# domargan/parallel-packed-csr

Hardware: AMD Instinct MI355X
Metric: edge-updates/sec (higher is better)
Workload: dtype u32; 1 GPU; config#2 1000000 random inserts on RMAT scale-20 / 10000000-edge core, 1 partition, labels raw; vertices=1048576, core_edges=10000000, parallelism=1 partition(s), 1 per GPU x 1 GPU(s), logN=32, distinct_update_batches=4, semantics=sequential stream order (bit-exact vs reference -threads=1)

## Files before the change

### parallel-packed-csr_amd/csrc/engine.cc

```cpp
#include "engine.h"

#include <stdio.h>
#include <stdlib.h>

#include <algorithm>
#include <map>
#include <memory>
#include <vector>
#include <chrono>

#include "gpu_rt.h"
#define GPU_DFREE(x) gpu::dfree_named((x), #x, __LINE__)
#include "pma_kernels.h"

namespace ppcsr {

#define GCHK(expr)                                                                       \
  do {                                                                                   \
    int _e = (expr);                                                                     \
    if (_e != 0) return fail(PPCSR_EHIP, std::string(#expr) + ": " + gpu::err_str(_e)); \
  } while (0)

struct DevGuard {
  std::vector<void **> slots;
// ... 39 lines not shown
  uint64_t rank_cap = 0, tiles_cap = 0;
  unsigned long long *d_total = nullptr, *h_total = nullptr;
  ChainTable *d_table = nullptr;
  unsigned long long *d_scan_state = nullptr;
  uint64_t scan_state_cap = 0, scan_nchunks = 0;
  Edge *d_scratch = nullptr;
  uint64_t scratch_cap = 0;
  int *d_nbr = nullptr;
  uint64_t nbr_cap = 0;
  uint32_t round = 0;
  uint32_t max_horizon = 4096, min_horizon = 64, rounds_per_sync = 32, init_horizon = 256;
  gpu::Timer timer;
  EngineStats st{};
  struct Snap {
    View v{};
    uint64_t cap_slots = 0, cap_nodes = 0;
    bool valid = false;
    uint32_t synced = 0;
    uint64_t gen = 0;
  };
  Snap snap, esnap;
  uint32_t snap_grid = 4096;
  bool snap_count = false;
  uint64_t snap_ctr[6] = {0, 0, 0, 0, 0, 0};
  unsigned long long *d_snapcnt = nullptr;
  uint64_t scc_ctr[8] = {0, 0, 0, 0, 0, 0, 0, 0};
  uint64_t msf_ctr[8] = {0, 0, 0, 0, 0, 0, 0, 0};
  uint64_t ktruss_ctr[8] = {0, 0, 0, 0, 0, 0, 0, 0};
  uint64_t msbfs_ctr[8] = {0, 0, 0, 0, 0, 0, 0, 0};
  uint32_t msbfs_look = 1;
  uint32_t serial = 1;
  uint64_t array_gen = 1;
  bool stamps_clean = false;
  OptCtl *d_octl = nullptr, *h_octl = nullptr;
  uint32_t *d_vdbg = nullptr;
  uint32_t *d_status = nullptr, *d_carry0 = nullptr, *d_carry1 = nullptr;
  uint64_t carry_cap = 0, hslot_cap = 0;
  unsigned long long *d_regfail = nullptr, *d_pfail = nullptr;
  uint32_t *d_vws = nullptr, *d_vrs = nullptr;
  uint32_t *d_wstamp = nullptr, *d_rstamp = nullptr;
  uint32_t mode = 1;
  uint32_t epoch_ops = 1u << 20;
  uint32_t cur_epoch = 0;
  uint32_t epoch_short = 16384;
  uint32_t epoch_clean = 0, epoch_grow_after = 2;
  uint32_t epoch_adapt = 8, grow_eff = 2;
  uint64_t since_rollback = 0;
  double rb_dist = -1.0;
  uint32_t region_slots = 1024;
  uint32_t region_wide = 4096, region_calm = 8, region_eff = 0, region_clean = 0;
  uint32_t region_rare = 16384, region_rare_calm = 8, region_rare_dist = 65536;
  uint64_t region_rare_span = 0;
  uint32_t region_rare_cpr = 1536;
  double cpr_mean = -1.0;
  uint32_t resident_waves = 0;
  uint32_t opt_horizon = 6144;
  uint32_t start_horizon = 6144;
  uint32_t adaptive = 1;
  uint32_t rb_defer_table = 1u << 22;
  uint32_t scatter_blocks = 8192;
  uint32_t small_batch = 256;
  uint32_t excl_in_wave = 4096;
  uint32_t big_window = 32768, big_min = 256, big_grid = 64;
  dev::BigJob *d_jobs = nullptr;
  Edge *d_bigscratch = nullptr;
  uint64_t bigscratch_cap = 0;
// ... 479 lines not shown
  }
  if (k == "rb_prefetch") {
    p.rb_prefetch = value ? 1u : 0u;
    return PPCSR_OK;
  }
  if (k == "msbfs_look") {
    p.msbfs_look = value ? 1u : 0u;
    return PPCSR_OK;
  }
  if (k == "scatter_variant") {
    p.scatter_variant = value > 2 ? 2u : (uint32_t)value;
    return PPCSR_OK;
  }
  if (k == "adaptive") {
    p.adaptive = value != 0;
    return PPCSR_OK;
  }
  if (k == "resident_waves") {
    if (value < 0 || value > (1 << 20)) return fail(PPCSR_EINVAL, "resident_waves out of range");
    p.resident_waves = (uint32_t)value;
    return PPCSR_OK;
  }
  if (k == "start_horizon") {
    if (value < 1 || value > (1 << 20)) return fail(PPCSR_EINVAL, "start_horizon out of range");
    p.start_horizon = (uint32_t)value;
    return PPCSR_OK;
  }
  if (k == "test_block_rebalance") {
    const uint64_t ws = (uint64_t)value >> 32, wl = (uint64_t)value & 0xFFFFFFFFull;
    if (wl < 64 || (wl & (wl - 1)) || ws % wl || ws + wl > p.v.g.N || (wl >> p.v.g.sh) > dev::kBigLeaves) return fail(PPCSR_EINVAL, "bad window");
    gpu::set_device(device_);
    Edge *sc = nullptr;
    GCHK(gpu::dmalloc((void **)&sc, wl * sizeof(Edge)));
    GPU_LAUNCH(p.stream, k_block_rebalance, 1, dev::kBigThreads, p.v, ws, wl, sc);
    GCHK(gpu::sync(p.stream));
    GCHK(gpu::last_error());
    gpu::dfree(sc);
    return PPCSR_OK;
  }
  if (k == "marker") {
    gpu::set_device(device_);
    uint32_t *np_ = nullptr;
    switch (value) {
      case 0: GPU_LAUNCH(p.stream, k_mark_0, 1, 64, np_); break;
      case 1: GPU_LAUNCH(p.stream, k_mark_1, 1, 64, np_); break;
      case 2: GPU_LAUNCH(p.stream, k_mark_2, 1, 64, np_); break;
      case 3: GPU_LAUNCH(p.stream, k_mark_3, 1, 64, np_); break;
      case 4: GPU_LAUNCH(p.stream, k_mark_4, 1, 64, np_); break;
      case 5: GPU_LAUNCH(p.stream, k_mark_5, 1, 64, np_); break;
      case 6: GPU_LAUNCH(p.stream, k_mark_6, 1, 64, np_); break;
      case 7: GPU_LAUNCH(p.stream, k_mark_7, 1, 64, np_); break;
      default: return fail(PPCSR_EINVAL, "marker id must be 0..7");
    }
    return PPCSR_OK;
  }
  if (k == "epoch_short") {
    p.epoch_short = (uint32_t)std::max<int64_t>(64, value);
    return PPCSR_OK;
  }
  if (k == "epoch_adapt") {
    p.epoch_adapt = (uint32_t)std::max<int64_t>(0, std::min<int64_t>(value, 1024));
    return PPCSR_OK;
  }
  if (k == "epoch_grow_after") {
    p.epoch_grow_after = (uint32_t)std::max<int64_t>(1, value);
    return PPCSR_OK;
// ... 60 lines not shown
    bool &f;
    explicit InBatch(bool &x) : f(x) { f = true; }
    ~InBatch() { f = false; }
  } in_batch_guard(p.in_batch);
  const uint64_t kChunk = 1ull << 30;
  for (uint64_t off = 0; off < n; off += kChunk) {
    const uint64_t m = std::min(kChunk, n - off);
    const bool small = m <= p.small_batch;
    int rc;
    if (p.v.g.narrow == 0u) {
      rc = recheck_ranges();
      if (rc != PPCSR_OK) return rc;
    }
    if (p.v.g.narrow == 0u) {
      const uint32_t mh = p.max_horizon, mi = p.min_horizon, ih = p.init_horizon;
      p.max_horizon = p.min_horizon = p.init_horizon = 1;
      rc = run_rounds(d_ops + off, m);
      p.max_horizon = mh;
      p.min_horizon = mi;
      p.init_horizon = ih;
    } else {
      rc = (p.mode == 1 && !small) ? run_speculative(d_ops + off, m) : run_rounds(d_ops + off, m);
    }
    if (rc != PPCSR_OK) return rc;
  }
  p.timer.stop(p.stream);
  p.st.last_batch_ms = p.timer.ms();
  p.st.ops_applied += n;
  return inplace_fault_check();
}

int Engine::run_rounds(const Op *d_ops, uint64_t n) {
  Impl &p = *p_;
  if (p.round > 0xFFFF0000u) GCHK(reset_tags(p));
  GCHK(ensure_plans(p));
  uint64_t cur = 0;
  uint32_t hor = (uint32_t)std::min<uint64_t>(p.init_horizon, n);
  while (cur < n) {
    const uint32_t par = (p.round + 1) & 1u;
    Control &c = *p.h_ctl;
    c.base[par] = (uint32_t)cur;
    c.base[par ^ 1u] = (uint32_t)cur;
    c.horizon[par] = (uint32_t)std::min<uint64_t>(hor, n - cur);
    c.horizon[par ^ 1u] = 0;
    c.failmin[0] = c.failmin[1] = kMax;
    c.n_ops = (uint32_t)n;
    c.excl = 0;
    c.error = 0;
    c.max_horizon = p.max_horizon;
    c.rounds = c.committed = c.planned = 0;
    GCHK(gpu::h2d(p.d_ctl, p.h_ctl, sizeof(Control), p.stream));
    bool need_excl = false;
    while (cur < n && !need_excl) {
      RoundArgs a;
      a.v = p.v;
      a.ops = d_ops;
      a.plans = p.d_plans;
      a.ctl = p.d_ctl;
      a.stats = p.d_stats;
      a.min_horizon = p.min_horizon;
      const uint32_t blocks = (p.max_horizon + 3) / 4;
      if (p.profile && p.events.size() < 4ull * p.rounds_per_sync) {
        const size_t old = p.events.size();
        p.events.resize(4ull * p.rounds_per_sync);
        for (size_t i = old; i < p.events.size(); i++) GCHK(p.events[i].init());
      }
// ... 21 lines not shown
          p.st.prof_plan_ms += gpu::Event::elapsed_ms(p.events[4 * r + 0], p.events[4 * r + 1]);
          p.st.prof_check_ms += gpu::Event::elapsed_ms(p.events[4 * r + 1], p.events[4 * r + 2]);
          p.st.prof_apply_ms += gpu::Event::elapsed_ms(p.events[4 * r + 2], p.events[4 * r + 3]);
          p.st.prof_launches += 1;
        }
      }
      p.st.round_syncs++;
      if (c.error) return fail(PPCSR_EINTERNAL, "device-side error " + std::to_string(c.error));
      const uint32_t npar = (p.round + 1) & 1u;
      cur = c.base[npar];
      hor = std::max<uint32_t>(c.horizon[npar], p.min_horizon);
      need_excl = c.excl != 0;
      p.st.rounds += c.rounds;
      p.st.committed += c.committed;
      p.st.planned += c.planned;
      c.rounds = c.committed = c.planned = 0;
      if (!need_excl && cur < n) {
        GCHK(gpu::dset(&p.d_ctl->rounds, 0, 3 * sizeof(unsigned long long), p.stream));
      }
    }
    if (need_excl && cur < n) {
      GCHK(gpu::d2h(p.h_op1, d_ops + cur, sizeof(Op), p.stream));
      GCHK(gpu::sync(p.stream));
      int rc = run_exclusive(*p.h_op1, 0);
      if (rc != PPCSR_OK) return rc;
      cur += 1;
    }
  }
  return PPCSR_OK;
}

static int snap_commit(Engine::Impl &p, Engine::Impl::Snap &sn);
static int snap_rollback(Engine::Impl &p, Engine::Impl::Snap &sn, Engine::Impl::Snap &other);

int Engine::run_speculative(const Op *d_ops, uint64_t n) {
  Impl &p = *p_;
  GCHK(ensure_plans(p));
  if (p.hslot_cap < p.opt_horizon) {
    if (p.d_status) GPU_DFREE(p.d_status);
    p.d_status = nullptr;
    p.hslot_cap = 0;
    GCHK(gpu::dmalloc((void **)&p.d_status, ((uint64_t)p.opt_horizon + 64) * sizeof(uint32_t)));
    if (p.d_vdbg) GPU_DFREE(p.d_vdbg);
    GCHK(gpu::dmalloc((void **)&p.d_vdbg, ((uint64_t)p.opt_horizon + 64) * 4 * sizeof(uint32_t)));
    p.hslot_cap = p.opt_horizon;
  }
  const uint64_t carry_need = (uint64_t)p.opt_horizon + 8;
  if (p.carry_cap < carry_need) {
    if (p.d_carry0) GPU_DFREE(p.d_carry0);
    if (p.d_carry1) GPU_DFREE(p.d_carry1);
    p.d_carry0 = p.d_carry1 = nullptr;
    p.carry_cap = 0;
    GCHK(gpu::dmalloc((void **)&p.d_carry0, kStripes * carry_need * sizeof(uint32_t)));
    GCHK(gpu::dmalloc((void **)&p.d_carry1, kStripes * carry_need * sizeof(uint32_t)));
    p.carry_cap = carry_need;
  }
  uint32_t bigw = p.big_window;
  while (bigw > kBigWindow && (bigw >> p.v.g.sh) > dev::kBigLeaves) bigw >>= 1;
  const bool use_big = bigw > p.big_min;
  if (use_big) {
    if (!p.d_jobs) GCHK(gpu::dmalloc((void **)&p.d_jobs, kBigJobs * sizeof(dev::BigJob)));
    const uint64_t need = (uint64_t)p.big_grid * bigw;
    if (p.bigscratch_cap < need) {
      if (p.d_bigscratch) GPU_DFREE(p.d_bigscratch);
      p.d_bigscratch = nullptr;
      p.bigscratch_cap = 0;
      GCHK(gpu::dmalloc((void **)&p.d_bigscratch, need * sizeof(Edge)));
      p.bigscratch_cap = need;
    }
  }
  if (p.diag >= 2) {
    if (p.dg_cap < n) {
      if (p.d_dg) GPU_DFREE(p.d_dg);
      p.d_dg = nullptr;
      p.dg_cap = 0;
      GCHK(gpu::dmalloc((void **)&p.d_dg, n * 4 * sizeof(uint32_t)));
      p.dg_cap = n;
    }
    GCHK(gpu::dset(p.d_dg, 0, n * 4 * sizeof(uint32_t), p.stream));
  }
  p.stamps_clean = false;
  uint64_t e0 = 0;
  uint64_t forced_e1 = 0;
  int retries = 0;
  const uint32_t kEpochShort = p.epoch_short;
  if (p.cur_epoch == 0 || p.cur_epoch > p.epoch_ops) p.cur_epoch = p.epoch_ops;
  while (e0 < n) {
    uint64_t e1 = std::min<uint64_t>(e0 + p.cur_epoch, n);
    if (forced_e1 > e0 && forced_e1 < e1) e1 = forced_e1;
    if (p.round > 0xFFFF0000u) GCHK(reset_tags(p));
    GCHK(snap_commit(p, p.esnap));
    GCHK(gpu::d2d(p.d_stats_snap, p.d_stats, kStatShards * sizeof(StatShard), p.stream));
    if (!p.stamps_clean) {
      const uint64_t leaves = p.v.g.N >> p.v.g.sh;
      GCHK(gpu::dset(p.d_wstamp, 0, leaves * sizeof(uint32_t), p.stream));
      GCHK(gpu::dset(p.d_rstamp, 0, leaves * sizeof(uint32_t), p.stream));
      GCHK(gpu::dset(p.d_vws, 0, (p.n_cap + 1) * sizeof(uint32_t), p.stream));
      GCHK(gpu::dset(p.d_vrs, 0, (p.n_cap + 1) * sizeof(uint32_t), p.stream));
      p.stamps_clean = true;
    }
    OptCtl &c = *p.h_octl;
    memset(&c, 0, sizeof(c));
    const uint32_t pp0 = p.round & 1u;
    c.hor[pp0] = 0;
    c.used[pp0] = 0;
    c.nf[pp0] = (uint32_t)e0;
    c.adaptive = p.adaptive;
    c.cur_h[pp0] = p.adaptive ? std::min(p.start_horizon, p.opt_horizon) : p.opt_horizon;
    c.book_round = p.round;
    for (int t = 0; t < 3; t++) {
      c.minkept[t] = kMax;
      c.gbar[t] = c.sbar[t] = ~0ull;
    }
    c.e1 = (uint32_t)e1;
    c.max_horizon = p.opt_horizon;
    c.width_cap = p.opt_horizon;
    c.resident = p.resident_waves;
    c.viol_idx = kMax;
    c.skip_idx = kMax;
    c.skip_round = 0;
    GCHK(gpu::h2d(p.d_octl, p.h_octl, sizeof(OptCtl), p.stream));
    int rs = 0;
    if (p.region_eff < p.region_slots) p.region_eff = p.region_slots;
    while ((p.region_eff >> rs) > (uint32_t)p.v.g.logN) rs++;
    bool epoch_open = true;
    uint32_t cur_width = c.cur_h[pp0];
    uint64_t carry_now = 0;
    unsigned long long jobs_seen = 0, rounds_seen = 0, planned_seen = 0, long_seen = 0;
    uint64_t chunk_pending = e1 - e0;
    double chunk_cpr = 0.9 * (double)std::min<uint64_t>(cur_width, e1 - e0);
    unsigned long long prev_rounds = 0, prev_committed = 0;
    uint32_t excl_cooldown = 0;
    while (epoch_open) {
      OptArgs a;
      a.v = p.v;
      a.v.big_window = use_big ? bigw : kBigWindow;
      a.big_min = p.big_min;
      a.jobs = use_big ? p.d_jobs : (dev::BigJob *)nullptr;
      a.bigscratch = p.d_bigscratch;
      a.bigscratch_stride = bigw;
      a.ops = d_ops;
      a.plans = p.d_plans;
      a.status = p.d_status;
      a.vdbg = p.d_vdbg;
      a.carry0 = p.d_carry0;
      a.carry1 = p.d_carry1;
      a.carry_cap = (uint32_t)p.carry_cap;
      a.ctl = p.d_octl;
      a.stats = p.d_stats;
      a.regfail = p.d_regfail;
      a.pfail = p.d_pfail;
      a.wstamp = p.d_wstamp;
      a.rstamp = p.d_rstamp;
      a.vws = p.d_vws;
      a.vrs = p.d_vrs;
      a.regshift = rs;
      a.diag = p.diag;
      a.defer_barrier = p.defer_barrier;
      const bool extras = p.diag != 0 || p.dbg_repeat != 0;
      a.dbg = p.dbg_repeat;
      a.dg = p.diag >= 2 ? p.d_dg : (uint32_t *)nullptr;
      a.soft_barrier = p.soft_barrier ? p.soft_barrier : a.v.big_window / 2u;
      if (!p.soft_barrier && p.region_rare_span && p.region_eff >= p.region_rare) a.soft_barrier = 0x40000000u;
      uint32_t gh = p.opt_horizon;
      {
        const uint64_t want = std::max<uint64_t>(1024, 4ull * (cur_width ? cur_width : p.opt_horizon));
        if (want < gh) gh = (uint32_t)want;
        const uint64_t pend = (chunk_pending + 255) & ~255ull;
        if (pend < gh) gh = (uint32_t)std::max<uint64_t>(pend, 256);
        const uint64_t need = (carry_now + 255) & ~255ull;
        if (gh < need) gh = (uint32_t)std::min<uint64_t>(need, p.opt_horizon);
      }
      const uint32_t blocks = (gh + 3) / 4;
      if (gh != c.max_horizon) {
        GCHK(gpu::h2d(&p.d_octl->max_horizon, &gh, sizeof(uint32_t), p.stream));
        c.max_horizon = gh;
      }
      uint32_t rounds = p.rounds_per_sync;
      {
        const double per_round = std::max(1.0, 0.85 * chunk_cpr);
        const double est = (double)chunk_pending / per_round + 2.0;
        if (est < (double)rounds) rounds = (uint32_t)std::max(2.0, est);
      }
      if (excl_cooldown) {
        rounds = std::min<uint32_t>(rounds, 8u);
        excl_cooldown--;
      }
      if (p.profile && p.events.size() < 5ull * rounds) {
        const size_t oldn = p.events.size();
        p.events.resize(5ull * rounds);
        for (size_t i = oldn; i < p.events.size(); i++) GCHK(p.events[i].init());
      }
      for (uint32_t r = 0; r < rounds; r++) {
        a.round = ++p.round;
        if (p.profile) p.events[5 * r + 0].record(p.stream);
        if (extras) GPU_LAUNCH(p.stream, o_plan_x, blocks, 256, a); else GPU_LAUNCH(p.stream, o_plan, blocks, 256, a);
        if (p.profile) p.events[5 * r + 1].record(p.stream);
        if (extras) GPU_LAUNCH(p.stream, o_check_x, blocks, 256, a);
        else if (p.check_force >= 0 ? p.check_force == 1 : p.check_lanes) GPU_LAUNCH(p.stream, o_check, (gh + kCkThreads - 1) / kCkThreads, kCkThreads, a);
        else GPU_LAUNCH(p.stream, o_check_w, blocks, 256, a);
        if (p.profile) p.events[5 * r + 2].record(p.stream);
        if (extras) GPU_LAUNCH(p.stream, o_apply_x, blocks, 256, a); else GPU_LAUNCH(p.stream, o_apply, blocks, 256, a);
        if (p.profile) p.events[5 * r + 3].record(p.stream);
        if (use_big && p.big_on) GPU_LAUNCH(p.stream, o_big, p.big_grid, 1024, a);
        if (p.profile) p.events[5 * r + 4].record(p.stream);
      }
      {
        a.round = p.round + 1;
        GPU_LAUNCH(p.stream, o_settle, 1, 64, a);
      }
      GCHK(gpu::d2h(p.h_octl, p.d_octl, sizeof(OptCtl), p.stream));
      GCHK(gpu::sync(p.stream));
      GCHK(gpu::last_error());
      if (p.profile) {
        for (uint32_t r = 0; r < rounds; r++) {
          p.st.prof_plan_ms += gpu::Event::elapsed_ms(p.events[5 * r + 0], p.events[5 * r + 1]);
          p.st.prof_check_ms += gpu::Event::elapsed_ms(p.events[5 * r + 1], p.events[5 * r + 2]);
          p.st.prof_apply_ms += gpu::Event::elapsed_ms(p.events[5 * r + 2], p.events[5 * r + 3]);
          if (use_big && p.big_on) p.st.prof_compact_ms += gpu::Event::elapsed_ms(p.events[5 * r + 3], p.events[5 * r + 4]);
          p.st.prof_launches += 1;
        }
      }
      p.st.round_syncs++;
      if (c.error) return fail(PPCSR_EINTERNAL, "device-side error " + std::to_string(c.error));
      {
// ... 40 lines not shown
        const uint64_t cnt = e1 - e0;
        std::vector<uint32_t> tr(cnt * 4);
        std::vector<Op> hops(cnt);
        GCHK(gpu::d2h(tr.data(), p.d_dg + 4 * e0, cnt * 4 * sizeof(uint32_t), p.stream));
        GCHK(gpu::d2h(hops.data(), d_ops + e0, cnt * sizeof(Op), p.stream));
        GCHK(gpu::sync(p.stream));
        if (FILE *f = fopen(getenv("PPCSR_DIAG_DUMP"), "ab")) {
          const uint64_t hdr[4] = {e0, e1, c.rounds, c.violation ? 1ull : 0ull};
          fwrite(hdr, sizeof(hdr), 1, f);
          fwrite(tr.data(), sizeof(uint32_t), tr.size(), f);
          fwrite(hops.data(), sizeof(Op), hops.size(), f);
          fclose(f);
        }
        GCHK(gpu::dset(p.d_dg + 4 * e0, 0, cnt * 4 * sizeof(uint32_t), p.stream));
      }
      const uint32_t npar = (c.book_round + 1u) & 1u;
      bool excl_resized = false;
      if (c.excl && !c.violation) {
        const uint64_t g = c.excl_idx;
        bool viol = false;
        int rc = run_exclusive(Op{0, 0, 0}, 0, d_ops, (uint32_t)g, &viol, &excl_resized, c.excl_later != 0);
        if (rc != PPCSR_OK) return rc;
        if (viol) {
          c.violation = 1;
          c.viol_idx = c.excl_idx;
        }
      }
      if (c.violation) {
        p.st.rollbacks++;
        if (getenv("PPCSR_TRACE_EPOCH"))
          fprintf(stderr, "[ppcsr] rollback: epoch [%llu,%llu) viol_idx=%u excl=%u later=%u after %llu rounds; kind=%u leaf=%u stamp=%u what=%u wleaf=[%u,%u] index=%u nr=%u\n",
                  (unsigned long long)e0, (unsigned long long)e1, c.viol_idx, c.excl, c.excl_later, c.rounds, c.viol_info[0],
                  c.viol_info[1], c.viol_info[2], c.viol_info[3], c.viol_info[4], c.viol_info[5], c.viol_info[6], c.viol_info[7]);
        GCHK(snap_rollback(p, p.esnap, p.snap));
        p.stamps_clean = false;
        GCHK(gpu::d2d(p.d_stats, p.d_stats_snap, kStatShards * sizeof(StatShard), p.stream));
        p.st.wasted_rounds += c.rounds;
        uint32_t short_eff = kEpochShort;
        p.grow_eff = p.epoch_grow_after;
        if (p.epoch_adapt) {
          const double D = (double)std::min<uint64_t>(p.since_rollback, 64ull * kEpochShort);
          p.rb_dist = p.rb_dist < 0 ? 64.0 * kEpochShort : (D < p.rb_dist ? 0.25 * p.rb_dist + 0.75 * D : 0.5 * p.rb_dist + 0.5 * D);
          p.since_rollback = 0;
          uint32_t q = 2048;
          while (2ull * q <= (uint64_t)(p.rb_dist / (double)p.epoch_adapt) && 2ull * q <= kEpochShort) q *= 2;
          short_eff = std::min<uint32_t>(kEpochShort, q);
          if (short_eff < kEpochShort) p.grow_eff = std::max<uint32_t>(p.epoch_grow_after, 4u);
        }
        p.cur_epoch = std::min<uint32_t>(p.cur_epoch, std::min<uint32_t>(p.epoch_ops, short_eff));
        p.epoch_clean = 0;
        {
          const bool rare = p.epoch_adapt && p.region_rare && p.rb_dist >= (double)p.region_rare_dist && p.cpr_mean >= (double)p.region_rare_cpr;
          p.region_eff = std::max(p.region_slots, rare ? std::max(p.region_wide, p.region_rare) : p.region_wide);
          p.region_rare_span = rare ? (uint64_t)(p.region_rare_calm * p.rb_dist) : 0;
        }
        p.region_clean = 0;
        const uint64_t cut = (uint64_t)c.viol_idx + 1;
        if (retries < 3 && c.viol_idx != kMax && cut > e0 && cut < e1) {
          retries++;
          forced_e1 = cut;
        } else {
          int rc = run_rounds(d_ops + e0, e1 - e0);
          if (rc != PPCSR_OK) return rc;
          e0 = e1;
          retries = 0;
          forced_e1 = 0;
        }
// ... 32 lines not shown
          const double cpr = (double)c.committed / (double)c.rounds;
          p.cpr_mean = p.cpr_mean < 0 ? cpr : 0.75 * p.cpr_mean + 0.25 * cpr;
        }
        e0 = e1;
        retries = 0;
        epoch_open = false;
        if (p.region_eff != p.region_slots) {
          ++p.region_clean;
          if (p.region_rare_span ? p.since_rollback >= p.region_rare_span : p.region_clean >= p.region_calm) {
            p.region_eff = p.region_slots;
            p.region_rare_span = 0;
          }
        }
        if (++p.epoch_clean >= std::max(p.grow_eff, p.epoch_grow_after)) {
          p.cur_epoch = (uint32_t)std::min<uint64_t>(p.epoch_ops, 2ull * p.cur_epoch);
          p.epoch_clean = 0;
        }
        if (c.cur_h[npar]) p.start_horizon = c.cur_h[npar];
      } else {
        cur_width = c.cur_h[npar];
        carry_now = c.used[npar];
        chunk_pending = (uint64_t)c.used[npar] + (uint64_t)(c.e1 - c.nf[npar]);
        if (c.rounds > prev_rounds) chunk_cpr = (double)(c.committed - prev_committed) / (double)(c.rounds - prev_rounds);
        prev_rounds = c.rounds;
        prev_committed = c.committed;
      }
    }
  }
  return PPCSR_OK;
}

int Engine::run_exclusive(Op op, uint32_t flags, const Op *d_ops, uint32_t spec_index, bool *violation, bool *resized, bool later_committed) {
  Impl &p = *p_;
  if (violation) *violation = false;
  if (resized) *resized = false;
  const bool spec = spec_index != kMax;
  bool counted = false;
  auto count_once = [&]() {
    if (!counted) p.st.exclusive_ops++;
    counted = true;
  };
  for (int attempt = 0; attempt < 8; attempt++) {
    XValid xv;
    xv.wstamp = p.d_wstamp;
    xv.rstamp = p.d_rstamp;
    xv.vws = p.d_vws;
    xv.me1 = (spec && attempt == 0) ? spec_index + 1u : 0u;
    const auto tx0 = std::chrono::steady_clock::now();
    GPU_LAUNCH(p.stream, k_exclusive, 1, 64, p.v, op, d_ops, spec ? spec_index : kMax, flags, p.d_xout, p.d_stats, p.excl_in_wave, xv);
    GCHK(gpu::d2h(p.h_xout, p.d_xout, sizeof(ExclOut), p.stream));
    GCHK(gpu::sync(p.stream));
    GCHK(gpu::last_error());
    const ExclOut x = *p.h_xout;
    if (getenv("PPCSR_TRACE_EXCL"))
      fprintf(stderr, "[excl] op (%u,%u,%u) flags %u -> result %u window (%u,%u) found %u, %.0f us\n", op.src, op.dst, op.op, flags, x.result, x.wstart, x.wlen, x.found,
              std::chrono::duration<double, std::micro>(std::chrono::steady_clock::now() - tx0).count());
    switch (x.result) {
      case X_DONE:
        count_once();
        return PPCSR_OK;
      case X_VIOLATION:
        if (violation) *violation = true;
        return PPCSR_OK;
      case X_NEED_DOUBLE:
      case X_NEED_HALF:
        if (spec && later_committed) {
// ... 55 lines not shown
    GCHK(gpu::dmalloc((void **)&p.d_rank, nleaves * sizeof(uint32_t)));
    p.rank_cap = nleaves;
  }
  return ensure_tiles((nleaves + kScanTile - 1) / kScanTile);
}

int Engine::ensure_tiles(uint64_t ntiles) {
  Impl &p = *p_;
  if (ntiles > p.tiles_cap) {
    if (p.d_tiles) GPU_DFREE(p.d_tiles);
    p.d_tiles = nullptr;
    p.tiles_cap = 0;
    GCHK(gpu::dmalloc((void **)&p.d_tiles, ntiles * sizeof(uint32_t)));
    p.tiles_cap = ntiles;
  }
  return PPCSR_OK;
}

int Engine::rank_scan(const uint32_t *d_cnt, uint64_t nleaves, bool table, uint64_t tb_index, uint64_t tb_len) {
  Impl &p = *p_;
  int rc = ensure_scratch(nleaves);
  if (rc != PPCSR_OK) return rc;
  const uint64_t ntiles = (nleaves + kScanTile - 1) / kScanTile;
  GPU_LAUNCH(p.stream, k_scan_tiles, ntiles, 256, d_cnt, nleaves, p.d_tiles);
  GPU_LAUNCH(p.stream, k_scan_tilesums, 1, kTileSumThreads, p.d_tiles, ntiles, p.d_total, table ? p.d_table : (ChainTable *)nullptr, tb_index, tb_len, (uint32_t *)nullptr, (uint32_t *)nullptr, 0u, 0u);
  GPU_LAUNCH(p.stream, k_scan_apply, ntiles, 256, d_cnt, nleaves, (const uint32_t *)p.d_tiles, p.d_rank);
  return PPCSR_OK;
}

int Engine::rebalance_fused(const View &nv, const Edge *src_items, uint64_t src_lo, uint64_t src_len, int src_sh,
                            uint32_t *src_cnt, bool inplace, uint64_t tb_index, uint64_t tb_len, Edge *dst, uint64_t dst_bias,
                            uint32_t *dst_cnt, uint64_t dst_nleaves) {
  Impl &p = *p_;
  const uint64_t nleaves = src_len >> src_sh;
  uint32_t tile = p.rb_tile;
  if (tile == 0) {
    tile = kRbTile;
    while (tile > 32 && nleaves / tile < p.rb_min_tiles) tile >>= 1;
  }
  const uint32_t lpc = 64u >> src_sh;
  if (tile < lpc) tile = lpc;
  if (tile > kRbTile) tile = kRbTile;
  const uint64_t ntiles = (nleaves + tile - 1) / tile;
  int rc = ensure_scratch(nleaves);
  if (rc == PPCSR_OK) rc = ensure_tiles(ntiles);
  if (rc != PPCSR_OK) return rc;
  const int dsh = nv.g.sh;
  GPU_LAUNCH(p.stream, k_rb_tilesums, ntiles, 256, src_cnt, nleaves, tile, p.d_tiles, inplace ? p.d_rank : (uint32_t *)nullptr,
             inplace ? (uint32_t *)nullptr : dst_cnt, inplace ? (uint64_t)0 : dst_nleaves,
             inplace ? p.v.ldirty + (src_cnt - p.v.leafcnt) : (uint32_t *)nullptr, p.serial);
  const uint32_t defer = (p.rb_defer_table && tb_index == 0 && tb_len >= (uint64_t)p.rb_defer_table) ? 1u : 0u;
  GPU_LAUNCH(p.stream, k_scan_tilesums, 1, kTileSumThreads, p.d_tiles, ntiles, p.d_total, p.d_table, tb_index, tb_len, (uint32_t *)nullptr, (uint32_t *)nullptr, 0u, defer);
  GPU_LAUNCH(p.stream, k_rb_scatter, ntiles, 256, nv, src_items, src_lo, src_len, src_sh,
               inplace ? (const uint32_t *)p.d_rank : (const uint32_t *)src_cnt, tile, p.rb_prefetch ? 4u : 1u, (const uint32_t *)p.d_tiles,
               p.d_table, dst, dst_bias, dst_cnt, nv.g.sh, (uint64_t)0, defer);
  return PPCSR_OK;
}

int Engine::resize(uint64_t newN) {
  Impl &p = *p_;
  if (newN < 2) return fail(PPCSR_EUNSUPPORTED, "array cannot shrink further");
  if (newN > (1ull << 31)) return fail(PPCSR_EUNSUPPORTED, "edge array would exceed 2^31 slots (reference indexes with int)");
  const View old = p.v;
  const uint64_t oldN = old.g.N;
  const uint64_t old_leaves = oldN >> old.g.sh;
  Geometry g;
  compute_geometry(newN, old.g.n, old.g.lock_search, &g);
  g.narrow = old.g.narrow;
  View nv = old;
  nv.g = g;
  const uint64_t new_leaves = newN >> g.sh;
  nv.items = nullptr;
  nv.leafcnt = nullptr;
  DevGuard guard;
  guard.add(&nv.items);
  guard.add(&nv.leafcnt);
  GCHK(gpu::dmalloc((void **)&nv.items, newN * sizeof(Edge)));
  GCHK(gpu::dmalloc((void **)&nv.leafcnt, new_leaves * sizeof(uint32_t)));
  int rc = PPCSR_OK;
  if (p.time_resize) p.timer.start(p.stream);
  if (p.scatter_variant == 2 && old.g.logN <= 32) {
    rc = rebalance_fused(nv, old.items, 0, oldN, old.g.sh, old.leafcnt, false, 0, newN, nv.items, 0, nv.leafcnt, new_leaves);
    if (rc != PPCSR_OK) return rc;
  } else {
    rc = rank_scan(old.leafcnt, old_leaves, true, 0, newN);
    if (rc != PPCSR_OK) return rc;
    GCHK(gpu::dset(nv.leafcnt, 0, new_leaves * sizeof(uint32_t), p.stream));
  }
  if (p.scatter_variant == 2 && old.g.logN <= 32) {
  } else if (p.scatter_variant == 1)
    GPU_LAUNCH(p.stream, k_scatter_runs, grid_for((oldN + 63) / 64, 4, p.scatter_blocks), 256, nv, (const Edge *)old.items, (uint64_t)0, oldN,
               old.g.sh, (const uint32_t *)p.d_rank, (const ChainTable *)p.d_table, nv.items, (uint64_t)0, nv.leafcnt, nv.g.sh,
               (uint64_t)0);
  else
    GPU_LAUNCH(p.stream, k_scatter_fill, grid_for((oldN + 63) / 64, 4), 256, nv, (const Edge *)old.items, (uint64_t)0, oldN,
// ... 3 lines not shown
  GCHK(gpu::sync(p.stream));
  GCHK(gpu::last_error());
  if (p.time_resize) p.last_resize_ms = p.timer.ms();
  guard.dismiss();
  GPU_DFREE(old.items);
  GPU_DFREE(old.leafcnt);
  {
    View tmp = old;
    free_aux(p, tmp);
  }
  p.v = nv;
  p.v.wres = p.v.rres = p.v.dres = nullptr;
  GCHK(alloc_aux(p, p.v));
  p.array_gen++;
  if (newN > oldN) p.st.double_calls++; else p.st.half_calls++;
  p.st.redistribute_calls++;
  p.st.redistribute_slots += newN;
  return PPCSR_OK;
}

int Engine::inplace_fault_check() {
  Impl &p = *p_;
  if (!p.ip_used) return PPCSR_OK;
  uint32_t err = 0;
  GCHK(gpu::d2h(&err, p.d_ip + 1, sizeof(uint32_t), p.stream));
  GCHK(gpu::sync(p.stream));
  p.ip_used = false;
  if (err) return fail(PPCSR_EINTERNAL, "in-place window rebalance: a tile waited for a source tile that never reported (tile order invalid)");
  return PPCSR_OK;
}

int Engine::big_redistribute(uint64_t wstart, uint64_t wlen, bool sync) {
  Impl &p = *p_;
  const View v = p.v;
  const uint64_t leaf_lo = wstart >> v.g.sh, nleaves = wlen >> v.g.sh;
  const bool fused = p.scatter_variant == 2 && v.g.logN <= 32;
  int rc = fused ? ensure_scratch(nleaves) : rank_scan(v.leafcnt + leaf_lo, nleaves, true, wstart, wlen);
  if (rc != PPCSR_OK) return rc;
  const bool whole = (wstart == 0 && wlen == v.g.N);
  if (fused && !whole && p.rb_inplace_min && wlen >= p.rb_inplace_min) {
    const uint32_t cpw = p.rb_inplace_cpw ? p.rb_inplace_cpw : ((wlen / 2048u <= kIpMaxTiles) ? 8u : 16u);
    const uint32_t tile_slots = 4u * cpw * 64u;
    const uint32_t tile_leaves = tile_slots >> v.g.sh;
    const uint64_t ntiles = wlen / tile_slots;
    if (ntiles >= 1 && ntiles <= kIpMaxTiles && wlen % tile_slots == 0 && tile_leaves >= 1 && tile_leaves <= kRbTile && (64u >> v.g.sh) >= 1u) {
      rc = ensure_tiles(ntiles);
      if (rc != PPCSR_OK) return rc;
      if (++p.ip_epoch == 0) {
        GCHK(gpu::dset(p.d_ip + kIpHdrWords + kIpMaxTiles, 0, (uint64_t)kIpMaxTiles * sizeof(uint32_t), p.stream));
        p.ip_epoch = 1;
      }
      uint32_t *order = p.d_ip + kIpHdrWords, *flags = p.d_ip + kIpHdrWords + kIpMaxTiles;
      GPU_LAUNCH(p.stream, k_rb_tilesums, ntiles, 256, v.leafcnt + leaf_lo, nleaves, tile_leaves, p.d_tiles, p.d_rank, (uint32_t *)nullptr, (uint64_t)0,
                 v.ldirty + leaf_lo, p.serial);
      GPU_LAUNCH(p.stream, k_scan_tilesums, 1, kTileSumThreads, p.d_tiles, ntiles, p.d_total, p.d_table, wstart, wlen, order, p.d_ip, tile_slots, 0u);
      if (cpw == 8)
        GPU_LAUNCH(p.stream, k_rb_inplace8, ntiles, 256, v, wstart, wlen, v.g.sh, (const uint32_t *)p.d_rank, (const uint32_t *)p.d_tiles,
                   (const ChainTable *)p.d_table, (const uint32_t *)order, p.d_ip, flags, p.ip_epoch, p.ip_lists);
      else
        GPU_LAUNCH(p.stream, k_rb_inplace16, ntiles, 256, v, wstart, wlen, v.g.sh, (const uint32_t *)p.d_rank, (const uint32_t *)p.d_tiles,
                   (const ChainTable *)p.d_table, (const uint32_t *)order, p.d_ip, flags, p.ip_epoch, p.ip_lists);
      p.ip_used = true;
      if (sync) {
        GCHK(gpu::sync(p.stream));
        GCHK(gpu::last_error());
        rc = inplace_fault_check();
// ... 22 lines not shown
  } else if (p.scatter_variant == 1)
    GPU_LAUNCH(p.stream, k_scatter_runs, grid_for((wlen + 63) / 64, 4, p.scatter_blocks), 256, v, (const Edge *)v.items, wstart, wlen, v.g.sh,
               (const uint32_t *)p.d_rank, (const ChainTable *)p.d_table, p.d_scratch, wstart, v.leafcnt, v.g.sh, (uint64_t)0);
  else
    GPU_LAUNCH(p.stream, k_scatter_fill, grid_for((wlen + 63) / 64, 4), 256, v, (const Edge *)v.items, wstart, wlen, v.g.sh,
               (const uint32_t *)p.d_rank, (const ChainTable *)p.d_table, p.d_scratch, wstart, v.leafcnt, v.g.sh, (uint64_t)0);
  if (whole) {
    std::swap(p.v.items, p.d_scratch);
  } else {
    GPU_LAUNCH(p.stream, k_copy_slots, grid_for(wlen * 3, 256 * 8), 256, (const Edge *)p.d_scratch, v.items + wstart, wlen);
  }
  if (sync) {
    GCHK(gpu::sync(p.stream));
    GCHK(gpu::last_error());
  }
  p.st.big_redistributes++;
  return PPCSR_OK;
}

int Engine::add_edge(uint32_t s, uint32_t d, uint32_t value) {
  if (value == 0) return PPCSR_OK;
  Op op{s, d, value};
  return apply_batch_host(&op, 1);
}
int Engine::remove_edge(uint32_t s, uint32_t d) {
  if (s >= n()) return fail(PPCSR_EINVAL, "remove_edge: src out of range (undefined behaviour in the reference)");
  Op op{s, d, 0};
  return apply_batch_host(&op, 1);
}

int Engine::add_node() {
  Impl &p = *p_;
  GCHK(gpu::set_device(device_));
  const uint32_t len = p.v.g.n;
  if ((uint64_t)len + 1 > p.n_cap) {
    const uint64_t ncap = p.n_cap * 2;
    Node *nn = nullptr;
    GCHK(gpu::dmalloc((void **)&nn, ncap * sizeof(Node)));
    GCHK(gpu::d2d(nn, p.v.nodes, (uint64_t)len * sizeof(Node), p.stream));
    GCHK(gpu::sync(p.stream));
    GPU_DFREE(p.v.nodes);
    p.v.nodes = nn;
    p.n_cap = ncap;
    GCHK(alloc_vertex_aux(p, p.v));
  }
  Node nd;
  uint32_t sval = len;
  if (len > 0) {
    Node last;
    GCHK(gpu::d2h(&last, p.v.nodes + (len - 1), sizeof(Node), p.stream));
    GCHK(gpu::sync(p.stream));
    nd.beginning = last.end;
    nd.end = nd.beginning + 1;
  } else {
    nd.beginning = 0;
    nd.end = 1;
    sval = kMax;
  }
  nd.num_neighbors = 0;
  GCHK(gpu::h2d(p.v.nodes + len, &nd, sizeof(Node), p.stream));
  GCHK(gpu::sync(p.stream));
  p.v.g.n = len + 1;
  p.array_gen++;
  Op op{len, nd.beginning, sval};
  const int rc = run_exclusive(op, XF_ADD_NODE | XF_FORCE_NOINFO);
  if (rc != PPCSR_OK) {
// ... 284 lines not shown
  while (tile > 16 && nchunks / tile < p.rb_min_tiles) tile >>= 1;
  const uint64_t ntiles = (nchunks + tile - 1) / tile;
  int rc = part->ensure_tiles(ntiles);
  if (rc != PPCSR_OK) return fail(rc, part->last_error());
  if (fresh_state) GCHK(gpu::dset(d_cs, 0, nchunks * sizeof(uint32_t), st));
  GPU_LAUNCH(st, k_chunk_sentinels, grid_for(p.v.g.n, 256), 256, p.v, d_cs);
  GPU_LAUNCH(st, k_chunk_counts, ntiles, 256, p.v, d_cs, d_cc, tile, p.d_tiles);
  GPU_LAUNCH(st, k_scan_tilesums, 1, kTileSumThreads, p.d_tiles, ntiles, p.d_total, (ChainTable *)nullptr, (uint64_t)0, (uint64_t)0, (uint32_t *)nullptr, (uint32_t *)nullptr, 0u, 0u);
  *tile_out = tile;
  *ntiles_out = ntiles;
  return PPCSR_OK;
}
void Engine::scan_write(Engine *part, uint32_t tile, uint64_t ntiles, unsigned long long *d_rows, int *d_dst, uint64_t cap, const float *d_values,
                        float *d_contrib, Op *d_triples, uint32_t src_base, uint32_t dest_bound) {
  Impl &p = *part->p_;
  const uint32_t *d_cc = reinterpret_cast<const uint32_t *>(p.d_scan_state) + p.scan_nchunks;
  GPU_LAUNCH(p_->stream, k_scan_write, ntiles, 256, p.v, d_cc, tile, (const uint32_t *)p.d_tiles, d_rows, d_dst, cap, d_values, d_contrib,
             d_triples, src_base, dest_bound);
}

int Engine::export_num_neighbors_device(uint32_t base, Op *d_out) {
  Impl &p = *p_;
  GCHK(gpu::set_device(device_));
  if (n() == 0) return PPCSR_OK;
  GPU_LAUNCH(p.stream, k_nn_export, grid_for(n(), 256), 256, p.v, base, d_out);
  GCHK(gpu::sync(p.stream));
  GCHK(gpu::last_error());
  return PPCSR_OK;
}
int Engine::set_num_neighbors_device(const Op *d_recs, uint64_t cnt) {
  Impl &p = *p_;
  GCHK(gpu::set_device(device_));
  if (cnt == 0) return PPCSR_OK;
  GPU_LAUNCH(p.stream, k_nn_set, grid_for(cnt, 256), 256, p.v, d_recs, cnt);
  GCHK(gpu::sync(p.stream));
  GCHK(gpu::last_error());
  return PPCSR_OK;
}
int Engine::export_triples_device(uint32_t src_base, Op *d_out, uint64_t cap, uint64_t *total) {
  Impl &p = *p_;
  GCHK(gpu::set_device(device_));
  int rc = scan_launch(nullptr, nullptr, d_out ? cap : 0, nullptr, nullptr, d_out, src_base);
  if (rc != PPCSR_OK) return rc;
  GCHK(gpu::d2h(p.h_total, p.d_total, sizeof(unsigned long long), p.stream));
  Edge last = null_edge();
  GCHK(gpu::d2h(&last, p.v.items + (p.v.g.N - 1), sizeof(Edge), p.stream));
  GCHK(gpu::sync(p.stream));
  GCHK(gpu::last_error());
  uint64_t tot = *p.h_total;
  if (last.value != 0 && !is_sentinel(last)) {
    if (d_out && tot < cap) {
      const Op o{last.src + src_base, last.dest, last.value};
      GCHK(gpu::h2d(d_out + tot, &o, sizeof(Op), p.stream));
      GCHK(gpu::sync(p.stream));
    }
    tot++;
  }
  if (total) *total = tot;
  return (d_out && tot > cap) ? PPCSR_ERANGE : PPCSR_OK;
}

template <class K, class V, class Tmp>
static int sort_pairs_stable(gpu::stream_t st, K *kin, K *kout, V *vin, V *vout, uint64_t m, unsigned bits, Tmp tmp) {
#if defined(PPCSR_SIM)
  (void)st;
  (void)bits;
  (void)tmp;
  std::vector<uint64_t> idx(m);
  for (uint64_t i = 0; i < m; i++) idx[i] = i;
  std::stable_sort(idx.begin(), idx.end(), [&](uint64_t a, uint64_t b) { return kin[a] < kin[b]; });
  for (uint64_t i = 0; i < m; i++) {
    kout[i] = kin[idx[i]];
    vout[i] = vin[idx[i]];
  }
  return 0;
#else
  size_t tmp_bytes = 0;
  if (rocprim::radix_sort_pairs(nullptr, tmp_bytes, kin, kout, vin, vout, (size_t)m, 0u, bits, st) != hipSuccess) return 3;
  void *t = tmp(tmp_bytes);
  if (!t) return 2;
  return rocprim::radix_sort_pairs(t, tmp_bytes, kin, kout, vin, vout, (size_t)m, 0u, bits, st) == hipSuccess ? 0 : 3;
#endif
}
template <class K, class V>
static int sort_pairs_stable(gpu::stream_t st, K *kin, K *kout, V *vin, V *vout, uint64_t m, unsigned bits) {
  void *t = nullptr;
  const int rc = sort_pairs_stable(st, kin, kout, vin, vout, m, bits, [&](size_t bytes) { return gpu::dmalloc(&t, bytes) == 0 ? t : nullptr; });
  if (t) {
    (void)gpu::sync(st);
    (void)gpu::dfree(t);
  }
  return rc;
}

int Engine::bulk_build(const Op *host_ops, uint64_t m, double *device_ms) { return bulk_build_from(host_ops, false, m, device_ms); }
int Engine::bulk_build_device(const Op *d_adds, uint64_t m, double *device_ms) { return bulk_build_from(d_adds, true, m, device_ms); }
int Engine::bulk_build_from(const Op *in_ops, bool on_device, uint64_t m, double *device_ms) {
  Impl &p = *p_;
  GCHK(gpu::set_device(device_));
  const uint32_t nn = n();
  if (nn == 0) return fail(PPCSR_EINVAL, "bulk_build: the graph has no vertices");
  if (m >= (1ull << 31)) return fail(PPCSR_EUNSUPPORTED, "bulk_build: too many edges for one call");
  {
    int rc = rank_scan(p.v.leafcnt, p.v.g.N >> p.v.g.sh, false, 0, 0);
    if (rc != PPCSR_OK) return rc;
    GCHK(gpu::d2h(p.h_total, p.d_total, sizeof(unsigned long long), p.stream));
    GCHK(gpu::sync(p.stream));
    if (*p.h_total != (unsigned long long)nn) return fail(PPCSR_EINVAL, "bulk_build: the graph already holds edges");
  }
  Op *d_ops = nullptr;
  unsigned long long *d_k0 = nullptr, *d_k1 = nullptr;
  uint32_t *d_v0 = nullptr, *d_v1 = nullptr, *d_flags = nullptr;
  DevGuard tmpg;
  tmpg.add(&d_ops); tmpg.add(&d_k0); tmpg.add(&d_k1); tmpg.add(&d_v0); tmpg.add(&d_v1); tmpg.add(&d_flags);
  const uint64_t mm = std::max<uint64_t>(m, 1);
  if (!on_device) GCHK(gpu::dmalloc((void **)&d_ops, mm * sizeof(Op)));
  GCHK(gpu::dmalloc((void **)&d_k0, mm * sizeof(unsigned long long)));
  GCHK(gpu::dmalloc((void **)&d_k1, mm * sizeof(unsigned long long)));
  GCHK(gpu::dmalloc((void **)&d_v0, mm * sizeof(uint32_t)));
  GCHK(gpu::dmalloc((void **)&d_v1, mm * sizeof(uint32_t)));
  GCHK(gpu::dmalloc((void **)&d_flags, mm * sizeof(uint32_t)));
  if (m && !on_device) GCHK(gpu::h2d(d_ops, in_ops, m * sizeof(Op), p.stream));
  const Op *src_ops = on_device ? in_ops : (const Op *)d_ops;
  p.timer.start(p.stream);
  uint64_t E = 0;
  if (m) {
    GPU_LAUNCH(p.stream, k_bb_keys, grid_for(m, 256), 256, src_ops, m, nn, d_k0, d_v0);
    unsigned bits = 1;
    while (bits < 32 && ((uint64_t)nn >> bits) != 0) bits++;
    int rc = sort_pairs_stable(p.stream, d_k0, d_k1, d_v0, d_v1, m, 32u + bits);
    if (rc != 0) return fail(rc == 2 ? PPCSR_ENOMEM : PPCSR_EHIP, "bulk_build: device sort failed");
    GPU_LAUNCH(p.stream, k_bb_flags, grid_for(m, 256), 256, (const unsigned long long *)d_k1, m, nn, d_flags);
// ... 258 lines not shown
    p.snap_ctr[0]++;
  } else {
    if ((e = snap_sync(p, sn, 0u, 0u))) return e;
    p.snap_ctr[2]++;
  }
  sn.synced = p.serial;
  advance_serial(p, 1);
  return 0;
}
static int snap_rollback(Engine::Impl &p, Engine::Impl::Snap &sn, Engine::Impl::Snap &other) {
  int e;
  if (!snap_in_step(p, sn)) {
    if ((e = snap_full_load(p, sn))) return e;
    p.snap_ctr[1]++;
    p.array_gen++;
    sn.gen = p.array_gen;
    other.gen = 0;
    sn.synced = p.serial;
    advance_serial(p, 1);
    return 0;
  }
  const uint32_t newtag = p.serial + 1u;
  if ((e = snap_sync(p, sn, newtag, 1u))) return e;
  p.snap_ctr[3]++;
  sn.synced = newtag;
  advance_serial(p, 2);
  return 0;
}

int Engine::snapshot() {
  Impl &p = *p_;
  GCHK(gpu::set_device(device_));
  GCHK(snap_commit(p, p.snap));
  GCHK(gpu::sync(p.stream));
  return PPCSR_OK;
}

int Engine::snap_counters(uint64_t out[6]) {
  if (!out) return fail(PPCSR_EINVAL, "snap counters: no output");
  for (int i = 0; i < 6; i++) out[i] = p_->snap_ctr[i];
  return PPCSR_OK;
}

int Engine::restore() {
  Impl &p = *p_;
  if (!p.snap.valid) return fail(PPCSR_EINVAL, "restore without snapshot");
  GCHK(gpu::set_device(device_));
  GCHK(snap_rollback(p, p.snap, p.esnap));
  p.stamps_clean = false;
  return PPCSR_OK;
}

int Engine::rebalance_bench(uint64_t wlen, int iters, double *ms_per_call) {
  Impl &p = *p_;
  if (wlen == 0 || wlen > p.v.g.N || (wlen & (wlen - 1)) || wlen < (uint64_t)p.v.g.logN) return fail(PPCSR_EINVAL, "bad window");
  GCHK(gpu::set_device(device_));
  const uint64_t wstart = p.rb_bench_upper ? p.v.g.N - wlen : 0;
  int rc = big_redistribute(wstart, wlen, true);
  if (rc != PPCSR_OK) return rc;
  p.timer.start(p.stream);
  for (int i = 0; i < iters; i++) {
    rc = big_redistribute(wstart, wlen, false);
    if (rc != PPCSR_OK) return rc;
  }
  p.timer.stop(p.stream);
  GCHK(gpu::sync(p.stream));
  GCHK(gpu::last_error());
  *ms_per_call = p.timer.ms() / iters;
#if defined(PPCSR_SCAN_DEBUG)
  {
    unsigned long long t[32];
    GCHK(gpu::d2h(t, p.d_total, sizeof(t), p.stream));
    GCHK(gpu::sync(p.stream));
    fprintf(stderr, "[scan] cycles: scan %llu, table %llu, order: table copy %llu, flags %llu, keys %llu, count %llu, hist scan %llu, scatter %llu (100 MHz ticks x ?)\n", t[9] - t[8], t[10] - t[9],
            t[11] - t[10], t[12] - t[11], t[13] - t[12], t[14] - t[13], t[15] - t[14], t[16] - t[15]);
  }
#endif
  return inplace_fault_check();
}

int Engine::chain_probe(const ChainProbeIO *io) {
// ... 440 lines not shown
```

### parallel-packed-csr_amd/csrc/pma_spec_rounds.h

```cpp
#pragma once
#include "pma_rounds.h"

namespace ppcsr {

constexpr uint32_t kStripes = 8;
struct OptCtl {
  uint32_t hor[2];
  uint32_t used[2];
  uint32_t nf[2];
  uint32_t cur_h[2];
  uint32_t kept[3][kStripes];
  uint32_t minkept[3];
  unsigned long long gbar[3];
  unsigned long long sbar[3];
  uint32_t njobs[3];
  uint32_t e1;
  uint32_t violation, excl, done, error;
  uint32_t max_horizon, excl_idx;
  uint32_t excl_later;
  uint32_t width_cap;
  uint32_t resident;
  uint32_t viol_idx;
  uint32_t adaptive;
  uint32_t book_round;
// ... 117 lines not shown
    c->committed += (unsigned long long)s.prev_committed;
    c->planned += (unsigned long long)s.prev_hor;
    c->jobs_total += (unsigned long long)s.prev_jobs;
  }
  c->hor[par] = s.hor;
  c->used[par] = s.used;
  c->nf[par] = s.nf;
  c->cur_h[par] = s.ch;
#pragma unroll
  for (uint32_t q = 0; q < kStripes; q++) c->kept[nt][q] = 0u;
  c->minkept[nt] = kMax;
  c->gbar[nt] = ~0ull;
  c->sbar[nt] = ~0ull;
  c->njobs[nt] = 0u;
  if (s.error) c->error = 77u;
  if (s.need_big) {
    c->need_big = 1u;
    return;
  }
  if (s.done) c->done = 1u;
  if (s.excl) {
    c->excl_idx = s.excl_idx;
    c->excl_later = s.excl_later;
    c->excl = 1u;
  }
}
PMA_KERNEL void o_settle(OptArgs a) {
  OptCtl *c = a.ctl;
  if (c->done || c->violation || c->excl || c->error || c->need_big) return;
  const RoundState s = round_begin(a, c);
  if (wv::thread_idx() == 0) round_record(a, c, s);
}

enum RoundWord : int { RW_STOP = 0, RW_HOR, RW_USED, RW_NF, RW_PRE0, RW_SKIP_IDX = RW_PRE0 + (int)kStripes + 1, RW_SKIP_ROUND, RW_WORDS };
static_assert(RW_WORDS <= 16, "round words");
template <bool EXTRAS>
PMA_DEV void o_plan_t(const OptArgs &a) {
  PMA_SHARED uint32_t rsh[16];
  OptCtl *c = a.ctl;
  const uint32_t rt = a.round % 3u;
  const int lane = wv::lane();
  const uint32_t wib = wv::uni((uint32_t)wv::wave_in_block());
  const uint32_t wid = wv::uni(wv::block_idx() * 4u) + wib;
  if (wib == 0u) {
    const uint32_t f_done = c->done, f_viol = c->violation, f_excl = c->excl, f_err = c->error | c->need_big;
    const uint32_t skip_idx = c->skip_idx, skip_round = c->skip_round;
    uint32_t stop = (f_done | f_viol | f_excl | f_err) ? 1u : 0u;
    uint32_t w = 0;
    if (!stop) {
      const RoundState rs = round_begin(a, c);
      if (wid == 0u && lane == 0) round_record(a, c, rs);
      stop = (rs.done | rs.excl | rs.error | rs.need_big) ? 1u : 0u;
      w = wv::setlane<RW_HOR>(w, rs.hor);
      w = wv::setlane<RW_USED>(w, rs.used);
      w = wv::setlane<RW_NF>(w, rs.nf);
      w = wv::setlane<RW_PRE0 + 0>(w, rs.pre[0]);
      w = wv::setlane<RW_PRE0 + 1>(w, rs.pre[1]);
      w = wv::setlane<RW_PRE0 + 2>(w, rs.pre[2]);
      w = wv::setlane<RW_PRE0 + 3>(w, rs.pre[3]);
      w = wv::setlane<RW_PRE0 + 4>(w, rs.pre[4]);
      w = wv::setlane<RW_PRE0 + 5>(w, rs.pre[5]);
      w = wv::setlane<RW_PRE0 + 6>(w, rs.pre[6]);
      w = wv::setlane<RW_PRE0 + 7>(w, rs.pre[7]);
      w = wv::setlane<RW_PRE0 + 8>(w, rs.pre[8]);
      w = wv::setlane<RW_SKIP_IDX>(w, skip_idx);
      w = wv::setlane<RW_SKIP_ROUND>(w, skip_round);
// ... 640 lines not shown
```

Measured before the change: 281.2 million edge-updates/s.

## Fuse epoch-begin memsets, stats copy and control upload into one kernel; skip redundant snapshot

At each speculative epoch start, the four stamp memsets, the stats-shard device copy and the OptCtl host-to-device upload are replaced by one k_epoch_begin kernel that receives the control block by value. The initial max_horizon is now computed with the same chunk-grid sizing used per chunk, so the later re-upload is less often needed. A live_is_snap flag tracks when the live array already equals the user snapshot, letting the epoch skip its own snapshot commit and roll back to the user snapshot instead. This cuts per-epoch launches and copies, at the cost of state tracking that every mutating path must reset correctly.

```diff
diff --git a/parallel-packed-csr_amd/csrc/engine.cc b/parallel-packed-csr_amd/csrc/engine.cc
--- a/parallel-packed-csr_amd/csrc/engine.cc
+++ b/parallel-packed-csr_amd/csrc/engine.cc
@@ -95,6 +95,7 @@
   uint32_t serial = 1;
   uint64_t array_gen = 1;
   bool stamps_clean = false;
+  bool live_is_snap = false;
   OptCtl *d_octl = nullptr, *h_octl = nullptr;
   uint32_t *d_vdbg = nullptr;
   uint32_t *d_status = nullptr, *d_carry0 = nullptr, *d_carry1 = nullptr;
@@ -640,6 +641,7 @@
     gpu::set_device(device_);
     Edge *sc = nullptr;
     GCHK(gpu::dmalloc((void **)&sc, wl * sizeof(Edge)));
+    p.live_is_snap = false;
     GPU_LAUNCH(p.stream, k_block_rebalance, 1, dev::kBigThreads, p.v, ws, wl, sc);
     GCHK(gpu::sync(p.stream));
     GCHK(gpu::last_error());
@@ -766,6 +768,7 @@
 
 int Engine::run_rounds(const Op *d_ops, uint64_t n) {
   Impl &p = *p_;
+  p.live_is_snap = false;
   if (p.round > 0xFFFF0000u) GCHK(reset_tags(p));
   GCHK(ensure_plans(p));
   uint64_t cur = 0;
@@ -853,6 +856,7 @@
 
 static int snap_commit(Engine::Impl &p, Engine::Impl::Snap &sn);
 static int snap_rollback(Engine::Impl &p, Engine::Impl::Snap &sn, Engine::Impl::Snap &other);
+static bool snap_in_step(const Engine::Impl &p, const Engine::Impl::Snap &sn);
 
 int Engine::run_speculative(const Op *d_ops, uint64_t n) {
   Impl &p = *p_;
@@ -910,16 +914,8 @@
     uint64_t e1 = std::min<uint64_t>(e0 + p.cur_epoch, n);
     if (forced_e1 > e0 && forced_e1 < e1) e1 = forced_e1;
     if (p.round > 0xFFFF0000u) GCHK(reset_tags(p));
-    GCHK(snap_commit(p, p.esnap));
-    GCHK(gpu::d2d(p.d_stats_snap, p.d_stats, kStatShards * sizeof(StatShard), p.stream));
-    if (!p.stamps_clean) {
-      const uint64_t leaves = p.v.g.N >> p.v.g.sh;
-      GCHK(gpu::dset(p.d_wstamp, 0, leaves * sizeof(uint32_t), p.stream));
-      GCHK(gpu::dset(p.d_rstamp, 0, leaves * sizeof(uint32_t), p.stream));
-      GCHK(gpu::dset(p.d_vws, 0, (p.n_cap + 1) * sizeof(uint32_t), p.stream));
-      GCHK(gpu::dset(p.d_vrs, 0, (p.n_cap + 1) * sizeof(uint32_t), p.stream));
-      p.stamps_clean = true;
-    }
+    const bool from_snap = p.live_is_snap && snap_in_step(p, p.snap);
+    if (!from_snap) GCHK(snap_commit(p, p.esnap));
     OptCtl &c = *p.h_octl;
     memset(&c, 0, sizeof(c));
     const uint32_t pp0 = p.round & 1u;
@@ -934,13 +930,30 @@
       c.gbar[t] = c.sbar[t] = ~0ull;
     }
     c.e1 = (uint32_t)e1;
-    c.max_horizon = p.opt_horizon;
     c.width_cap = p.opt_horizon;
     c.resident = p.resident_waves;
     c.viol_idx = kMax;
     c.skip_idx = kMax;
     c.skip_round = 0;
-    GCHK(gpu::h2d(p.d_octl, p.h_octl, sizeof(OptCtl), p.stream));
+    auto chunk_grid = [&p](uint32_t width, uint64_t pending, uint64_t carry) {
+      uint32_t gh = p.opt_horizon;
+      const uint64_t want = std::max<uint64_t>(1024, 4ull * (width ? width : p.opt_horizon));
+      if (want < gh) gh = (uint32_t)want;
+      const uint64_t pend = (pending + 255) & ~255ull;
+      if (pend < gh) gh = (uint32_t)std::max<uint64_t>(pend, 256);
+      const uint64_t need = (carry + 255) & ~255ull;
+      if (gh < need) gh = (uint32_t)std::min<uint64_t>(need, p.opt_horizon);
+      return gh;
+    };
+    c.max_horizon = chunk_grid(c.cur_h[pp0], e1 - e0, 0);
+    {
+      const uint64_t leaves = p.v.g.N >> p.v.g.sh, nv = (uint64_t)p.n_cap + 1;
+      const uint32_t clear = p.stamps_clean ? 0u : 1u;
+      const uint64_t quads = clear ? std::max(leaves, nv) / 4 + 1 : kStatShards * sizeof(StatShard) / 16;
+      GPU_LAUNCH(p.stream, k_epoch_begin, (uint32_t)std::min<uint64_t>((quads + 255) / 256, 2048), 256, p.d_wstamp, p.d_rstamp, leaves, p.d_vws, p.d_vrs, nv,
+                 clear, (const StatShard *)p.d_stats, p.d_stats_snap, p.d_octl, c);
+      p.stamps_clean = true;
+    }
     int rs = 0;
     if (p.region_eff < p.region_slots) p.region_eff = p.region_slots;
     while ((p.region_eff >> rs) > (uint32_t)p.v.g.logN) rs++;
@@ -983,15 +996,7 @@
       a.dg = p.diag >= 2 ? p.d_dg : (uint32_t *)nullptr;
       a.soft_barrier = p.soft_barrier ? p.soft_barrier : a.v.big_window / 2u;
       if (!p.soft_barrier && p.region_rare_span && p.region_eff >= p.region_rare) a.soft_barrier = 0x40000000u;
-      uint32_t gh = p.opt_horizon;
-      {
-        const uint64_t want = std::max<uint64_t>(1024, 4ull * (cur_width ? cur_width : p.opt_horizon));
-        if (want < gh) gh = (uint32_t)want;
-        const uint64_t pend = (chunk_pending + 255) & ~255ull;
-        if (pend < gh) gh = (uint32_t)std::max<uint64_t>(pend, 256);
-        const uint64_t need = (carry_now + 255) & ~255ull;
-        if (gh < need) gh = (uint32_t)std::min<uint64_t>(need, p.opt_horizon);
-      }
+      const uint32_t gh = chunk_grid(cur_width, chunk_pending, carry_now);
       const uint32_t blocks = (gh + 3) / 4;
       if (gh != c.max_horizon) {
         GCHK(gpu::h2d(&p.d_octl->max_horizon, &gh, sizeof(uint32_t), p.stream));
@@ -1012,6 +1017,7 @@
         p.events.resize(5ull * rounds);
         for (size_t i = oldn; i < p.events.size(); i++) GCHK(p.events[i].init());
       }
+      p.live_is_snap = false;
       for (uint32_t r = 0; r < rounds; r++) {
         a.round = ++p.round;
         if (p.profile) p.events[5 * r + 0].record(p.stream);
@@ -1118,7 +1124,12 @@
           fprintf(stderr, "[ppcsr] rollback: epoch [%llu,%llu) viol_idx=%u excl=%u later=%u after %llu rounds; kind=%u leaf=%u stamp=%u what=%u wleaf=[%u,%u] index=%u nr=%u\n",
                   (unsigned long long)e0, (unsigned long long)e1, c.viol_idx, c.excl, c.excl_later, c.rounds, c.viol_info[0],
                   c.viol_info[1], c.viol_info[2], c.viol_info[3], c.viol_info[4], c.viol_info[5], c.viol_info[6], c.viol_info[7]);
-        GCHK(snap_rollback(p, p.esnap, p.snap));
+        if (from_snap) {
+          GCHK(snap_rollback(p, p.snap, p.esnap));
+          p.live_is_snap = true;
+        } else {
+          GCHK(snap_rollback(p, p.esnap, p.snap));
+        }
         p.stamps_clean = false;
         GCHK(gpu::d2d(p.d_stats, p.d_stats_snap, kStatShards * sizeof(StatShard), p.stream));
         p.st.wasted_rounds += c.rounds;
@@ -1217,6 +1228,7 @@
 
 int Engine::run_exclusive(Op op, uint32_t flags, const Op *d_ops, uint32_t spec_index, bool *violation, bool *resized, bool later_committed) {
   Impl &p = *p_;
+  p.live_is_snap = false;
   if (violation) *violation = false;
   if (resized) *resized = false;
   const bool spec = spec_index != kMax;
@@ -1338,6 +1350,7 @@
                             uint32_t *src_cnt, bool inplace, uint64_t tb_index, uint64_t tb_len, Edge *dst, uint64_t dst_bias,
                             uint32_t *dst_cnt, uint64_t dst_nleaves) {
   Impl &p = *p_;
+  p.live_is_snap = false;
   const uint64_t nleaves = src_len >> src_sh;
   uint32_t tile = p.rb_tile;
   if (tile == 0) {
@@ -1367,6 +1380,7 @@
   Impl &p = *p_;
   if (newN < 2) return fail(PPCSR_EUNSUPPORTED, "array cannot shrink further");
   if (newN > (1ull << 31)) return fail(PPCSR_EUNSUPPORTED, "edge array would exceed 2^31 slots (reference indexes with int)");
+  p.live_is_snap = false;
   const View old = p.v;
   const uint64_t oldN = old.g.N;
   const uint64_t old_leaves = oldN >> old.g.sh;
@@ -1436,6 +1450,7 @@
 
 int Engine::big_redistribute(uint64_t wstart, uint64_t wlen, bool sync) {
   Impl &p = *p_;
+  p.live_is_snap = false;
   const View v = p.v;
   const uint64_t leaf_lo = wstart >> v.g.sh, nleaves = wlen >> v.g.sh;
   const bool fused = p.scatter_variant == 2 && v.g.logN <= 32;
@@ -1524,6 +1539,7 @@
 int Engine::add_node() {
   Impl &p = *p_;
   GCHK(gpu::set_device(device_));
+  p.live_is_snap = false;
   const uint32_t len = p.v.g.n;
   if ((uint64_t)len + 1 > p.n_cap) {
     const uint64_t ncap = p.n_cap * 2;
@@ -1874,6 +1890,7 @@
   Impl &p = *p_;
   GCHK(gpu::set_device(device_));
   if (cnt == 0) return PPCSR_OK;
+  p.live_is_snap = false;
   GPU_LAUNCH(p.stream, k_nn_set, grid_for(cnt, 256), 256, p.v, d_recs, cnt);
   GCHK(gpu::sync(p.stream));
   GCHK(gpu::last_error());
@@ -1940,6 +1957,7 @@
 int Engine::bulk_build_from(const Op *in_ops, bool on_device, uint64_t m, double *device_ms) {
   Impl &p = *p_;
   GCHK(gpu::set_device(device_));
+  p.live_is_snap = false;
   const uint32_t nn = n();
   if (nn == 0) return fail(PPCSR_EINVAL, "bulk_build: the graph has no vertices");
   if (m >= (1ull << 31)) return fail(PPCSR_EUNSUPPORTED, "bulk_build: too many edges for one call");
@@ -2264,6 +2282,7 @@
   Impl &p = *p_;
   GCHK(gpu::set_device(device_));
   GCHK(snap_commit(p, p.snap));
+  p.live_is_snap = true;
   GCHK(gpu::sync(p.stream));
   return PPCSR_OK;
 }
@@ -2279,6 +2298,7 @@
   if (!p.snap.valid) return fail(PPCSR_EINVAL, "restore without snapshot");
   GCHK(gpu::set_device(device_));
   GCHK(snap_rollback(p, p.snap, p.esnap));
+  p.live_is_snap = true;
   p.stamps_clean = false;
   return PPCSR_OK;
 }
diff --git a/parallel-packed-csr_amd/csrc/pma_spec_rounds.h b/parallel-packed-csr_amd/csrc/pma_spec_rounds.h
--- a/parallel-packed-csr_amd/csrc/pma_spec_rounds.h
+++ b/parallel-packed-csr_amd/csrc/pma_spec_rounds.h
@@ -173,6 +173,31 @@
   if (wv::thread_idx() == 0) round_record(a, c, s);
 }
 
+PMA_DEV void epoch_zero_words(uint32_t *p, uint64_t n, uint64_t tid, uint64_t stride) {
+  uint4 *p4 = reinterpret_cast<uint4 *>(p);
+  const uint64_t n4 = n >> 2;
+  uint4 z;
+  z.x = z.y = z.z = z.w = 0u;
+  for (uint64_t i = tid; i < n4; i += stride) p4[i] = z;
+  if (tid < (n & 3ull)) p[(n4 << 2) + tid] = 0u;
+}
+PMA_KERNEL void k_epoch_begin(uint32_t *wstamp, uint32_t *rstamp, uint64_t leaves, uint32_t *vws, uint32_t *vrs, uint64_t nv, uint32_t clear,
+                              const StatShard *stats, StatShard *stats_snap, OptCtl *ctl, OptCtl init) {
+  const uint64_t stride = (uint64_t)wv::grid_dim() * wv::block_dim();
+  const uint64_t tid = (uint64_t)wv::block_idx() * wv::block_dim() + wv::thread_idx();
+  if (clear) {
+    epoch_zero_words(wstamp, leaves, tid, stride);
+    epoch_zero_words(rstamp, leaves, tid, stride);
+    epoch_zero_words(vws, nv, tid, stride);
+    epoch_zero_words(vrs, nv, tid, stride);
+  }
+  static_assert((kStatShards * sizeof(StatShard)) % sizeof(uint4) == 0, "stat shards: whole 16-byte words");
+  const uint4 *s4 = reinterpret_cast<const uint4 *>(stats);
+  uint4 *d4 = reinterpret_cast<uint4 *>(stats_snap);
+  for (uint64_t i = tid; i < kStatShards * sizeof(StatShard) / sizeof(uint4); i += stride) d4[i] = s4[i];
+  if (tid == 0) *ctl = init;
+}
+
 enum RoundWord : int { RW_STOP = 0, RW_HOR, RW_USED, RW_NF, RW_PRE0, RW_SKIP_IDX = RW_PRE0 + (int)kStripes + 1, RW_SKIP_ROUND, RW_WORDS };
 static_assert(RW_WORDS <= 16, "round words");
 template <bool EXTRAS>
```

Result: faster. 287.0 million edge-updates/s (median of 6 runs) (+2.1%).
